# Yixin-F/DR-Using-SCV-OD

Hardware: AMD Instinct MI355X
Metric: scans/sec on SemanticKITTI-seq-05-shaped input (SCV-OD dynamic-removal path, raw scans -> per-point labels + static map) (higher is better)
Workload: dtype f32

## Files before the change

### dr-using-scv-od_amd/csrc/scvod_k_voxels.inc

```
__global__ __launch_bounds__(256) void k_apri_expand(DevParams P, Arena A, int s0) {
    const int s = s0 + blockIdx.y;
    const int base = A.scan_off[s];
    const int n = A.counts[s * 8 + 4];
    for (int i = blockIdx.x * 256 + threadIdx.x; i < n; i += gridDim.x * 256) {
        const float4 q = A.pts[base + A.apri_src[(size_t)base + i]];
        Apri a;
        apri_of_point(P.bin, q.x, q.y, q.z, q.w, a);
        scvod_apri out;
        out.x = a.x;
        out.y = a.y;
        out.z = a.z;
        out.range = a.range;
        out.angle = a.angle;
        out.azimuth = a.azimuth;
        out.intensity = a.intensity;
        out.range_idx = a.range_idx;
        out.sector_idx = a.sector_idx;
        out.azimuth_idx = a.azimuth_idx;
        out.voxel_idx = a.voxel_idx;
        A.apri[(size_t)base + i] = out;
    }
}

__global__ __launch_bounds__(256) void k_cls_from_lists(Arena A, int s) {
    const int base = A.scan_off[s];
    const int n_g = A.counts[s * 8 + 1], n_ng = A.counts[s * 8 + 2];
    for (int i = blockIdx.x * 256 + threadIdx.x; i < n_g + n_ng; i += gridDim.x * 256) {
        if (i < n_g)
            A.cls[base + A.ground_idx[(size_t)base + i]] = SCVOD_CLS_GROUND;
        else
            A.cls[base + A.nonground_idx[(size_t)base + (i - n_g)]] = SCVOD_CLS_NONGROUND;
    }
}

__global__ __launch_bounds__(1024) void k_bin_direct(DevParams P, Arena A, int apply_filter) {
    __shared__ int wsum[17];
    const int s = blockIdx.x;
    const int base = A.scan_off[s];
    const int n = A.scan_off[s + 1] - base;
    int run = 0;
    for (int c0 = 0; c0 < n; c0 += 1024) {
        int i = c0 + threadIdx.x;
        int keep = 0;
        Apri a;
        if (i < n) {
            float4 q = A.pts[base + i];
            keep = apri_of_point(P.bin, q.x, q.y, q.z, q.w, a);
            if (!apply_filter) keep = 1;
        }
        int tk;
        int ek = block_excl_scan<1024>(keep, tk, wsum);
        if (i < n) {
            if (keep) {
                size_t dst = (size_t)base + run + ek;
                scvod_apri out;
                out.x = a.x;
                out.y = a.y;
                out.z = a.z;
                out.range = a.range;
                out.angle = a.angle;
                out.azimuth = a.azimuth;
                out.intensity = a.intensity;
                out.range_idx = a.range_idx;
                out.sector_idx = a.sector_idx;
                out.azimuth_idx = a.azimuth_idx;
                out.voxel_idx = a.voxel_idx;
                A.apri[dst] = out;
                A.apri_src[dst] = i;
                A.apri_key[dst] = a.voxel_idx;
                A.apri_int[dst] = a.intensity;
                A.apri_idx3[dst] = pack_idx3(a.range_idx, a.sector_idx, a.azimuth_idx);
            } else {
                A.rejected_src[(size_t)base + (i - (run + ek))] = i;
            }
        }
        run += tk;
    }
    if (threadIdx.x == 0) {
        A.scan_irr[s] = 0;
        A.irr_list[(size_t)s * (kIrrListCap + 1)] = -1;
        int* c = A.counts + s * 8;
        c[0] = n;
        c[1] = 0;
        c[2] = 0;
        c[3] = 0;
        c[4] = run;
        c[5] = n - run;
        c[6] = 0;
        c[7] = 0;
    }
}

__global__ __launch_bounds__(256) void k_apri_split(Arena A) {
    const int s = blockIdx.y;
    const int base = A.scan_off[s];
    const int n = A.counts[s * 8 + 4];
    for (int i = blockIdx.x * 256 + threadIdx.x; i < n; i += gridDim.x * 256) {
        const scvod_apri& a = A.apri[(size_t)base + i];
        A.apri_key[(size_t)base + i] = a.voxel_idx;
        A.apri_int[(size_t)base + i] = a.intensity;
        A.apri_idx3[(size_t)base + i] = pack_idx3(a.range_idx, a.sector_idx, a.azimuth_idx);
    }
}

__device__ __forceinline__ int vx_bucket_of(const DevParams& P, const Arena& A, int s, int32_t voxel_idx) {
    if (A.vb_lut) {
        if (voxel_idx == 0x7fffffff) return kMaxBuckets - 1;
        return A.vb_lut[(size_t)s * kVgLutBins + (voxel_idx >> *A.vb_lut_shift)];
    }
    int64_t b = ((int64_t)voxel_idx + P.key_off) >> P.vb_shift;
    if (b < 0) b = 0;
    if (b > P.n_buckets - 1) b = P.n_buckets - 1;
    return (int)b;
}
__device__ __forceinline__ uint32_t vx_bias(int32_t k) { return (uint32_t)k ^ 0x80000000u; }
__device__ __forceinline__ int32_t vx_unbias(uint32_t u) { return (int32_t)(u ^ 0x80000000u); }

__global__ __launch_bounds__(1024) void k_vx_partition(DevParams P, Arena A) {
    __shared__ int hist[kMaxBuckets];
    __shared__ int wsum[17];
    const int s = blockIdx.x;
    const int base = A.scan_off[s];
    const int n = A.counts[s * 8 + 4];
    const int tid = threadIdx.x;
    if (tid < kMaxBuckets) hist[tid] = 0;
    __syncthreads();
    constexpr int U = 4;
    for (int i0 = 0; i0 < n; i0 += 1024 * U) {
        int32_t key[U];
#pragma unroll
        for (int u = 0; u < U; ++u) key[u] = A.apri_key[(size_t)base + min(i0 + u * 1024 + tid, n - 1)];
#pragma unroll
        for (int u = 0; u < U; ++u) wave_bin_add(hist, i0 + u * 1024 + tid < n ? vx_bucket_of(P, A, s, key[u]) : -1);
    }
    __syncthreads();
    const int c = (tid < P.n_buckets) ? hist[tid] : 0;
    int total;
    const int ex = block_excl_scan<1024>(c, total, wsum);
    if (tid < kMaxBuckets) {
        A.vb_count[s * kMaxBuckets + tid] = c;
        hist[tid] = ex;
    }
    if (tid <= P.n_buckets) A.vb_off[s * (kMaxBuckets + 1) + tid] = ex;
    __syncthreads();
    for (int i0 = 0; i0 < n; i0 += 1024 * U) {
        int32_t key[U];
#pragma unroll
        for (int u = 0; u < U; ++u) key[u] = A.apri_key[(size_t)base + min(i0 + u * 1024 + tid, n - 1)];
#pragma unroll
        for (int u = 0; u < U; ++u) {
            const int i = i0 + u * 1024 + tid;
            const int bk = i < n ? vx_bucket_of(P, A, s, key[u]) : -1;
            const int at = wave_bin_rank(hist, bk);
            if (bk >= 0) {
                if (A.vx_k32)
                    ((uint32_t*)A.vkeys)[(size_t)base + at] = (uint32_t)((((int64_t)key[u] + P.key_off) & ((1ll << P.vb_shift) - 1)) << A.vx_idx_bits) | (uint32_t)i;
                else
                    A.vkeys[(size_t)base + at] = pack_key(vx_bias(key[u]), (uint32_t)i);
            }
        }
    }
}

#ifndef SCVOD_VOX_K32_LDS
#define SCVOD_VOX_K32_LDS 1
#endif
constexpr size_t vox_key_bytes(int cap, size_t ksize) { return (((size_t)(cap + cap / 8) * (SCVOD_VOX_K32_LDS ? ksize : 8)) + 15) & ~(size_t)15; }
constexpr size_t vox_aux_bytes(int cap, bool desc) { return desc ? (size_t)cap * 4 : ((size_t)(cap / 64) * 4 + 15) & ~(size_t)15; }
constexpr size_t vox_lds_bytes(int cap, size_t ksize = 8, bool desc = true) {
    return vox_key_bytes(cap, ksize) + (size_t)cap * 4 + vox_aux_bytes(cap, desc) + 128;
}
#ifndef SCVOD_VOX_LEAN_MORE
#define SCVOD_VOX_LEAN_MORE 4
#endif
#ifndef SCVOD_VOX_LEAN_S
#define SCVOD_VOX_LEAN_S 12
#endif
template <int U, typename F>
__device__ __forceinline__ void vx_descriptor(int n, F&& at, float& av_out, float& cov_out) {
    float av = 0.f;
    for (int j0 = 0; j0 < n; j0 += U) {
        float x[U];
#pragma unroll
        for (int u = 0; u < U; ++u) x[u] = (j0 + u < n) ? at(j0 + u) : 0.f;
#pragma unroll
        for (int u = 0; u < U; ++u)
            if (j0 + u < n) av += x[u];
    }
    const float fn = (float)n;
    av = av / fn;
    float cov = 0.f;
    for (int j0 = 0; j0 < n; j0 += U) {
        float x[U];
#pragma unroll
        for (int u = 0; u < U; ++u) x[u] = (j0 + u < n) ? at(j0 + u) : 0.f;
#pragma unroll
        for (int u = 0; u < U; ++u)
            if (j0 + u < n) {
                const double d = (double)(x[u] - av);
                cov = (float)((double)cov + d * d);
            }
    }
    av_out = av;
    cov_out = cov / fn;
}
constexpr bool vx_bucket_padfree(int cap) { return SCVOD_VOX_PADFREE == 2 || (SCVOD_VOX_PADFREE == 1 && cap >= 2048); }
template <int CAP, int THREADS, int C_LO, int C_HI, int LGE, int MODE = 0, typename KT = unsigned long long, bool DESC = true>
__global__ __launch_bounds__(THREADS)
#if SCVOD_VOX_K32_LDS
__attribute__((amdgpu_waves_per_eu((sizeof(KT) == 4 && CAP <= 4096 && CAP >= 2048) ? (DESC ? 6 : 2 * SCVOD_VOX_LEAN_MORE) : 1, 8)))
#endif
void k_vx_bucket(DevParams P, Arena A) {
    static_assert(DESC || MODE == 0, "the lean form is makeHashCloud's");
    extern __shared__ __attribute__((aligned(16))) unsigned char smem[];
    constexpr bool K32 = sizeof(KT) == 4;
    constexpr bool PADFREE = vx_bucket_padfree(CAP);
    constexpr bool PADK = true;
    constexpr int SLOTS = CAP + CAP / 8;
    KT* l_keys = (KT*)smem;
    constexpr size_t KB = vox_key_bytes(CAP, sizeof(KT));
    static_assert(KB >= (size_t)SLOTS * sizeof(KT), "key area");
    int* l_vbeg = (int*)(smem + KB);
    float* l_int = (float*)(smem + KB + (size_t)CAP * 4);
    int* wsum = (int*)(smem + KB + (size_t)CAP * 4 + vox_aux_bytes(CAP, DESC));
    int lo, hi;
    order_range(A.vorder_off, C_LO, C_HI, lo, hi);
    constexpr bool PV = (CAP == 4096 && MODE == 0);
    PROF_BEGIN();
    for (int w = lo + blockIdx.x; w < hi; w += gridDim.x) {
    if (PV) PROF_RESET();
    const int4 item = A.vorder[w];
    const int code = item.x;
    const int s = code / kMaxBuckets, b = code - s * kMaxBuckets;
    const int m = item.y;
    const int base = item.z, off = item.w;
    if (MODE == 1 && b == kMaxBuckets - 1) {
        if (threadIdx.x == 0) A.vb_nvox[s * kMaxBuckets + b] = 0;
        continue;
    }
    const bool in_lds = (m <= CAP);
    KT* keys;
    int* vbeg;
    float* ints;
    KT* gkeys = (KT*)A.vkeys + (size_t)base + off;
    const KT kpad = K32 ? (KT)0xffffffffu : (KT)kKeyPad;
    const uint32_t imask = (1u << A.vx_idx_bits) - 1u;
    auto k_major = [&](KT k) -> uint32_t { return K32 ? (uint32_t)k >> A.vx_idx_bits : key_major((unsigned long long)k); };
    auto k_idx = [&](KT k) -> uint32_t { return K32 ? (uint32_t)k & imask : key_idx((unsigned long long)k); };
    if (in_lds) {
        int np2 = 1 << LGE;
        while (np2 < m) np2 <<= 1;
        const int nlive = sortnet::live_end(m, LGE);
        constexpr int IT = CAP / THREADS;
        keys = l_keys;
        vbeg = l_vbeg;
        ints = l_int;
        bool from_regs = false;
        if constexpr (IT == (1 << LGE) && CAP >= 4096) {
            if (np2 == CAP) {
                from_regs = true;
                KT tmp[IT];
                if constexpr (PADFREE) {
                    if ((int)threadIdx.x < (nlive >> LGE)) {
#pragma unroll
                        for (int it = 0; it < IT; ++it) {
                            const int j = sortnet::start_key(it, (int)threadIdx.x, nlive, LGE);
                            tmp[it] = (j < m) ? gkeys[j] : kpad;
                        }
                    }
                    if (PV) PROF_MARK(3, 0);
                    padfree_sort_regs<THREADS, PADK, LGE>(tmp, keys, np2, nlive, kpad);
                } else {
#pragma unroll
                    for (int it = 0; it < IT; ++it) {
                        const int j = it * THREADS + (int)threadIdx.x;
                        tmp[it] = (j < m) ? gkeys[j] : kpad;
                    }
                    if (PV) PROF_MARK(3, 0);
                    block_bitonic_sort_pow2_regs<THREADS, PADK, LGE>(tmp, keys);
                }
            }
        }
        if (!from_regs) {
            const int nfill = PADFREE ? nlive : np2;
            for (int j = threadIdx.x; j < nfill; j += THREADS) l_keys[sort_slot<PADK>(j)] = (j < m) ? gkeys[j] : kpad;
            __syncthreads();
            if (PV) PROF_MARK(3, 0);
            if constexpr (PADFREE)
                padfree_sort<THREADS, PADK, LGE>(keys, np2, nlive, kpad);
            else
                block_bitonic_sort_pow2<THREADS, PADK, LGE>(keys, np2);
        }
        if (PV) PROF_MARK(3, 1);
    } else {
        keys = gkeys;
        vbeg = A.tmp_vox_begin + (size_t)base + off;
        ints = nullptr;
        block_bitonic_sort<THREADS, false>(keys, m);
    }
#define KX(j) (in_lds ? sort_slot<PADK>(j) : (j))
    int run = 0;
    if (in_lds) {
        constexpr int NW = THREADS / 64;
        static_assert(CAP / 64 <= 128, "two (chunk, wave) counts per lane");
        int* wcnt = (int*)l_int;
        const int lane = threadIdx.x & 63, wave = threadIdx.x >> 6;
        const int chunks = (m + THREADS - 1) / THREADS;
        auto head_of = [&](int j, KT& cur) -> bool {
            cur = keys[KX(j)];
            const KT prev = keys[KX(j > 0 ? j - 1 : 0)];
            return (j == 0) || (k_major(cur) != k_major(prev));
        };
        for (int c = 0; c < chunks; ++c) {
            const int j = c * THREADS + threadIdx.x;
            bool head = false;
            if (j < m) {
                KT cur;
                head = head_of(j, cur);
                if (MODE == 0) A.vox_pts[(size_t)base + off + j] = (int32_t)k_idx(cur);
            }
            const unsigned long long hb = __ballot(head);
            if (lane == 0) wcnt[c * NW + wave] = __popcll(hb);
        }
        __syncthreads();
        const int ne = chunks * NW;
        if (wave == 0) {
            const int a0 = (2 * lane < ne) ? wcnt[2 * lane] : 0, a1 = (2 * lane + 1 < ne) ? wcnt[2 * lane + 1] : 0;
            const int inc = wave_incl_scan(a0 + a1);
            if (2 * lane < ne) wcnt[2 * lane] = inc - a0 - a1;
            if (2 * lane + 1 < ne) wcnt[2 * lane + 1] = inc - a1;
            if (lane == 63) wsum[0] = inc;
        }
        __syncthreads();
        run = wsum[0];
        for (int c = 0; c < chunks; ++c) {
            const int j = c * THREADS + threadIdx.x;
            KT cur;
            const bool head = (j < m) && head_of(j, cur);
            const unsigned long long hb = __ballot(head);
            if (head) vbeg[wcnt[c * NW + wave] + __popcll(hb & ((1ull << lane) - 1ull))] = j;
        }
    }
    for (int c0 = 0; c0 < m && !in_lds; c0 += THREADS) {
        int j = c0 + threadIdx.x;
        int head = 0;
        if (j < m) {
            const KT cur = keys[KX(j)];
            const KT prev = keys[KX(j > 0 ? j - 1 : 0)];
            head = (j == 0) || (k_major(cur) != k_major(prev));
            const uint32_t idx = k_idx(cur);
            if (MODE == 0) A.vox_pts[(size_t)base + off + j] = (int32_t)idx;
        }
        int th;
        int eh = block_excl_scan<THREADS>(head, th, wsum);
        if (head) vbeg[run + eh] = j;
        run += th;
    }
    __syncthreads();
    if (PV) PROF_MARK(3, 2);
    const int nv = run;
    if (MODE == 1) {
        float4* tmp = (float4*)A.apri;
        for (int v = threadIdx.x; v < nv; v += THREADS) {
            const int j0 = vbeg[v];
            const int j1 = (v + 1 < nv) ? vbeg[v + 1] : m;
            float sx = 0.f, sy = 0.f, sz = 0.f, si = 0.f;
            for (int j = j0; j < j1; ++j) {
                const float4 p = A.pts[base + k_idx(keys[KX(j)])];
                sx += p.x;
                sy += p.y;
                sz += p.z;
                si += A.vg_labels ? p.w * A.vg_max_intensity : p.w;
            }
            const float fn = (float)(j1 - j0);
            tmp[(size_t)base + off + v] = make_float4(sx / fn, sy / fn, sz / fn, si / fn);
        }
        if (threadIdx.x == 0) A.vb_nvox[s * kMaxBuckets + b] = nv;
        __syncthreads();
        continue;
    }
    auto vox_key_of = [&](int j0) -> int32_t {
        return K32 ? (int32_t)(((int64_t)b << P.vb_shift) + (int64_t)k_major(keys[KX(j0)]) - P.key_off) : vx_unbias(k_major(keys[KX(j0)]));
    };
    if constexpr (DESC) {
        if (in_lds) {
            for (int j = threadIdx.x; j < m; j += THREADS) ints[j] = A.apri_int[(size_t)base + k_idx(keys[KX(j)])];
            __syncthreads();
        }
        if (PV) PROF_MARK(3, 3);
        for (int v = threadIdx.x; v < nv; v += THREADS) {
            const int j0 = vbeg[v];
            const int j1 = (v + 1 < nv) ? vbeg[v + 1] : m;
            float av, cov;
            if (in_lds)
                vx_descriptor<1>(j1 - j0, [&](int j) { return ints[j0 + j]; }, av, cov);
            else
                vx_descriptor<1>(j1 - j0, [&](int j) { return A.apri_int[(size_t)base + k_idx(keys[j0 + j])]; }, av, cov);
            A.tmp_vox_key[(size_t)base + off + v] = vox_key_of(j0);
            A.tmp_vox_cov[(size_t)base + off + v] = cov;
            A.tmp_vox_av[(size_t)base + off + v] = av;
        }
// ... 67 lines not shown
```

### dr-using-scv-od_amd/csrc/scvod_kernels.hip

```cpp
#include <type_traits>

#include "scvod_boxgrid.h"
#include "scvod_grid.h"
#include "scvod_sortnet.h"
#include <rocprim/device/device_radix_sort.hpp>

namespace scvod {

#ifdef SCVOD_PROFILE
__device__ unsigned long long g_prof[8][16];
#define PROF_BEGIN() unsigned long long t_prev = wall_clock64()
#define PROF_RESET()                                   \
    do {                                               \
        __syncthreads();                               \
        if (threadIdx.x == 0) t_prev = wall_clock64(); \
    } while (0)
#define PROF_MARK(k, i)                                      \
    do {                                                     \
        __syncthreads();                                     \
        if (threadIdx.x == 0) {                              \
            const unsigned long long t_now = wall_clock64(); \
            atomicAdd(&g_prof[k][i], t_now - t_prev);        \
            t_prev = t_now;                                  \
        }                                                    \
// ... 196 lines not shown

template <bool PAD, int LGE, typename T>
__device__ __forceinline__ void bitonic_run_to_lds(T (&e)[1 << LGE], T* a, int b) {
    constexpr int E = 1 << LGE;
#pragma unroll
    for (int kk = 2; kk <= E; kk <<= 1) {
#pragma unroll
        for (int d = kk >> 1; d >= 1; d >>= 1) {
#pragma unroll
            for (int m = 0; m < E; ++m)
                if ((m & d) == 0) {
                    if (kk == E || (m & kk) == 0)
                        cswap_asc(e[m], e[m + d]);
                    else
                        cswap_asc(e[m + d], e[m]);
                }
        }
    }
    const int rev = ((b & E) == 0) ? 0 : (E - 1);
#pragma unroll
    for (int m = 0; m < E; ++m) a[sort_slot<PAD>(b + (m ^ rev))] = e[m];
}

template <int THREADS, bool PAD, int LGE, typename T>
__device__ __forceinline__ void block_bitonic_merge_stages(T* a, int np2);

template <int THREADS, bool PAD, int LGE, typename T>
__device__ __forceinline__ void block_bitonic_sort_pow2(T* a, int np2) {
    constexpr int E = 1 << LGE;
    for (int g = threadIdx.x; g < (np2 >> LGE); g += THREADS) {
        const int b = g << LGE;
        T e[E];
#pragma unroll
        for (int m = 0; m < E; ++m) e[m] = a[sort_slot<PAD>(b + m)];
        bitonic_run_to_lds<PAD, LGE>(e, a, b);
    }
    __syncthreads();
    block_bitonic_merge_stages<THREADS, PAD, LGE>(a, np2);
}

template <int THREADS, bool PAD, int LGE, typename T>
__device__ __forceinline__ void block_bitonic_sort_pow2_regs(T (&e)[1 << LGE], T* a) {
    bitonic_run_to_lds<PAD, LGE>(e, a, (int)threadIdx.x << LGE);
    __syncthreads();
    block_bitonic_merge_stages<THREADS, PAD, LGE>(a, THREADS << LGE);
}

template <int THREADS, bool PAD, int LGE, typename T>
__device__ __forceinline__ void block_bitonic_merge_stages(T* a, int np2) {
    constexpr int E = 1 << LGE;
    int lgk = LGE + 1;
    for (int k = 2 * E; k <= np2; k <<= 1, ++lgk) {
        int r = lgk;
        const int first = (r % LGE) ? (r % LGE) : LGE;
        if (first == 1)
            bitonic_pass<THREADS, PAD, 1>(a, np2, k, r);
        else if (first == 2)
            bitonic_pass<THREADS, PAD, 2>(a, np2, k, r);
        else if (first == 3)
            bitonic_pass<THREADS, PAD, 3>(a, np2, k, r);
        else
            bitonic_pass<THREADS, PAD, 4>(a, np2, k, r);
        r -= first;
        while (r > 0) {
            bitonic_pass<THREADS, PAD, LGE>(a, np2, k, r);
            r -= LGE;
        }
    }
}

#ifndef SCVOD_SORT_PADFREE
#define SCVOD_SORT_PADFREE 1
#endif
#ifndef SCVOD_VOX_PADFREE
#define SCVOD_VOX_PADFREE 1
#endif
struct CxAsc {
    template <typename T>
    __device__ __forceinline__ void operator()(T& lo, T& hi) const { cswap_asc(lo, hi); }
};

template <int THREADS, bool PAD, int LT, bool MIRROR, typename T>
__device__ __forceinline__ void padfree_pass(T* a, int np2, int nlive, int r, T padv) {
    const int items = sortnet::pass_items(np2, nlive, r, LT);
    for (int t = threadIdx.x; t < items; t += THREADS) sortnet::pass_item<LT, MIRROR, PAD, T>(a, t, r, nlive, padv, CxAsc{});
    __syncthreads();
}

template <int THREADS, bool PAD, int LGE, typename T>
__device__ __forceinline__ void padfree_merge_stages(T* a, int np2, int nlive, T padv) {
    sortnet::for_each_pass<LGE>(np2, [&](int r, int lt, bool mirror) {
        if (!mirror)
            padfree_pass<THREADS, PAD, LGE, false>(a, np2, nlive, r, padv);
        else if (lt == 1)
            padfree_pass<THREADS, PAD, 1, true>(a, np2, nlive, r, padv);
        else if (lt == 2)
            padfree_pass<THREADS, PAD, 2, true>(a, np2, nlive, r, padv);
        else if (lt == 3 || LGE == 3)
            padfree_pass<THREADS, PAD, 3, true>(a, np2, nlive, r, padv);
        else if constexpr (LGE >= 4)
            padfree_pass<THREADS, PAD, 4, true>(a, np2, nlive, r, padv);
    });
}

template <int THREADS, bool PAD, int LGE, typename T>
__device__ __forceinline__ void padfree_sort(T* a, int np2, int nlive, T padv) {
    constexpr int E = 1 << LGE;
    for (int g = threadIdx.x; g < (nlive >> LGE); g += THREADS) {
        T e[E];
#pragma unroll
        for (int m = 0; m < E; ++m) e[m] = a[sort_slot<PAD>((g << LGE) + m)];
        sortnet::run_store<LGE, PAD>(e, a, g, CxAsc{});
    }
    __syncthreads();
    padfree_merge_stages<THREADS, PAD, LGE>(a, np2, nlive, padv);
}

template <int THREADS, bool PAD, int LGE, typename T>
__device__ __forceinline__ void padfree_sort_regs(T (&e)[1 << LGE], T* a, int np2, int nlive, T padv) {
    if ((int)threadIdx.x < (nlive >> LGE)) sortnet::run_store<LGE, PAD>(e, a, (int)threadIdx.x, CxAsc{});
    __syncthreads();
    padfree_merge_stages<THREADS, PAD, LGE>(a, np2, nlive, padv);
}

#include "scvod_k_patchwork.inc"
#include "scvod_k_voxelgrid.inc"
#include "scvod_k_voxels.inc"
#include "scvod_k_cluster.inc"
#include "scvod_k_merge.inc"
#include "scvod_k_rgrow.inc"
#include "scvod_k_calib.inc"
#include "scvod_k_probe_nn.inc"
#define TH_BEGIN(name) \
    if (th) th(tu, name, 1)
#define TH_END(name) \
    if (th) th(tu, name, 0)

#ifndef SCVOD_SORT_LGE
#define SCVOD_SORT_LGE 4
#endif
constexpr int kLGE = SCVOD_SORT_LGE;
constexpr int kTS = (kLGE == 4) ? 1 : 2;
#ifndef SCVOD_VOX_LGE
#define SCVOD_VOX_LGE 3
#endif
constexpr int kLGEv = SCVOD_VOX_LGE, kTSv = (kLGEv == 4) ? 1 : 2;
constexpr int kPersistCUs = 256;
constexpr int kSortCapS = 1024, kSortThreadsS = 64;
constexpr int kSortCapL = 8192, kSortThreadsL = 512;
constexpr int kSortCapXL = 16384, kClassXL = 52;
constexpr size_t sort_lds_bytes(int cap) { return (size_t)(cap + cap / 8) * 8; }
constexpr int kVoxCapS = 1024, kVoxThreadsS = 64;
constexpr int kVoxCapL = 8192, kVoxThreadsL = 512;

void launch_process(const DevParams& P, const Arena& A, hipStream_t st, int do_patchwork, int apply_filter,
                    int do_voxels, TimerHook th, void* tu, int lean_voxels, int lean_emit) {
    const int B = A.n_scans;
    if (B <= 0) return;
    if (do_patchwork == 1) {
        hipMemsetAsync(A.patch_count, 0, sizeof(int32_t) * (size_t)B * kMaxPatches, st);
        hipMemsetAsync(A.patch_cursor, 0, sizeof(int32_t) * (size_t)B * kMaxPatches, st);
        dim3 gcls((A.max_scan_pts + kClsThreads * kClsItems - 1) / (kClsThreads * kClsItems), B);
        TH_BEGIN("pw_classify");
        hipLaunchKernelGGL(k_pw_classify, gcls, dim3(kClsThreads), 0, st, P, A);
        TH_END("pw_classify");
        TH_BEGIN("pw_offsets");
        hipLaunchKernelGGL(k_pw_offsets, dim3(B), dim3(1024), 0, st, P, A);
        TH_END("pw_offsets");
        TH_BEGIN("pw_scatter");
        hipLaunchKernelGGL(k_pw_scatter, gcls, dim3(kClsThreads), 0, st, P, A);
        TH_END("pw_scatter");
        hipMemsetAsync(A.order_hist, 0, sizeof(int32_t) * 64, st);
        hipMemsetAsync(A.order_cursor, 0, sizeof(int32_t) * 64, st);
        const int n_all = B * P.n_patches;
        TH_BEGIN("pw_order");
        hipLaunchKernelGGL(k_pw_order_count, dim3((n_all + 255) / 256), dim3(256), 0, st, P, A);
        hipLaunchKernelGGL(k_pw_order_offsets, dim3(1), dim3(64), 0, st, A);
        hipLaunchKernelGGL(k_pw_order_scatter, dim3((n_all + 255) / 256), dim3(256), 0, st, P, A);
        TH_END("pw_order");
        hipFuncSetAttribute((const void*)k_pw_sort<kSortCapXL, 1024, kClassXL, 63, 4>, hipFuncAttributeMaxDynamicSharedMemorySize,
                            (int)sort_lds_bytes(kSortCapXL));
        hipFuncSetAttribute((const void*)k_pw_sort<kSortCapL, kSortThreadsL * kTS, kClassL, kClassXL - 1, kLGE>,
                            hipFuncAttributeMaxDynamicSharedMemorySize, (int)sort_lds_bytes(kSortCapL));
        TH_BEGIN("pw_sort_8192");
        hipLaunchKernelGGL((k_pw_sort<kSortCapXL, 1024, kClassXL, 63, 4>), dim3(kPersistCUs), dim3(1024), sort_lds_bytes(kSortCapXL), st, P, A);
        hipLaunchKernelGGL((k_pw_sort<kSortCapL, kSortThreadsL * kTS, kClassL, kClassXL - 1, kLGE>), dim3(kPersistCUs * 2),
                           dim3(kSortThreadsL * kTS), sort_lds_bytes(kSortCapL), st, P, A);
        TH_END("pw_sort_8192");
        TH_BEGIN("pw_sort_4096");
        hipLaunchKernelGGL((k_pw_sort<4096, 256 * kTS, kClassM2, kClassL - 1, kLGE>), dim3(kPersistCUs * 4), dim3(256 * kTS),
                           sort_lds_bytes(4096), st, P, A);
        TH_END("pw_sort_4096");
        TH_BEGIN("pw_sort_2048");
        hipLaunchKernelGGL((k_pw_sort<2048, 128 * kTS, kClassM, kClassM2 - 1, kLGE>), dim3(kPersistCUs * 8), dim3(128 * kTS),
                           sort_lds_bytes(2048), st, P, A);
        TH_END("pw_sort_2048");
        TH_BEGIN("pw_sort_1024");
        hipLaunchKernelGGL((k_pw_sort<kSortCapS, kSortThreadsS * kTS, kClassXS, kClassM - 1, kLGE>), dim3(kPersistCUs * 16),
                           dim3(kSortThreadsS * kTS), sort_lds_bytes(kSortCapS), st, P, A);
        TH_END("pw_sort_1024");
        TH_BEGIN("pw_sort_256");
        hipLaunchKernelGGL((k_pw_sort<256, 64, kClassWave, kClassXS - 1, 3>), dim3(kPersistCUs * 32), dim3(64),
                           sort_lds_bytes(256), st, P, A);
        TH_END("pw_sort_256");
        TH_BEGIN("pw_sort_wave");
        hipLaunchKernelGGL(k_pw_sort_wave, dim3(kPersistCUs * 8), dim3(256), 0, st, P, A);
        TH_END("pw_sort_wave");
        const int coop_class = (B <= 8) ? kClassWave : kClassFitCoop;
        const int coop_min = 1 << (coop_class / 4);
        TH_BEGIN("pw_fit_large");
        const dim3 gfit((int)(A.total_pts / coop_min / (B <= 8 ? 1 : 4)) + 1);
        if (B <= 8) {
            if (lean_emit)
                hipLaunchKernelGGL((k_pw_fit_coop<64, true>), gfit, dim3(64), 0, st, P, A, coop_class);
            else
                hipLaunchKernelGGL((k_pw_fit_coop<64, false>), gfit, dim3(64), 0, st, P, A, coop_class);
        } else {
            if (lean_emit)
                hipLaunchKernelGGL((k_pw_fit_coop<16, true>), gfit, dim3(64), 0, st, P, A, coop_class);
            else
                hipLaunchKernelGGL((k_pw_fit_coop<16, false>), gfit, dim3(64), 0, st, P, A, coop_class);
        }
        TH_END("pw_fit_large");
        TH_BEGIN("pw_fit");
        hipLaunchKernelGGL(k_pw_fit, dim3((n_all + 63) / 64), dim3(64), 0, st, P, A, coop_class);
        TH_END("pw_fit");
        TH_BEGIN("pw_arrange");
        if (lean_emit) {
            if (coop_class > kClassWave) hipLaunchKernelGGL((k_pw_arrange<64, true>), dim3(kPersistCUs * 8), dim3(256), 0, st, P, A, kClassWave, coop_class - 1);
            hipLaunchKernelGGL((k_pw_arrange<16, true>), dim3(kPersistCUs * 4), dim3(256), 0, st, P, A, 0, kClassWave - 1);
        } else {
            if (coop_class > kClassWave) hipLaunchKernelGGL((k_pw_arrange<64, false>), dim3(kPersistCUs * 8), dim3(256), 0, st, P, A, kClassWave, coop_class - 1);
            hipLaunchKernelGGL((k_pw_arrange<16, false>), dim3(kPersistCUs * 4), dim3(256), 0, st, P, A, 0, kClassWave - 1);
        }
        TH_END("pw_arrange");
        TH_BEGIN("emit_offsets");
        hipLaunchKernelGGL(k_emit_offsets, dim3(B), dim3(1024), 0, st, P, A);
        TH_END("emit_offsets");
        TH_BEGIN("emit");
        if (lean_emit)
            hipLaunchKernelGGL(k_emit<true>, dim3(kPersistCUs * 8), dim3(kEmitThreads), 0, st, P, A);
        else
            hipLaunchKernelGGL(k_emit<false>, dim3(kPersistCUs * 8), dim3(kEmitThreads), 0, st, P, A);
        TH_END("emit");
    } else if (do_patchwork == 0) {
        TH_BEGIN("bin_direct");
        hipLaunchKernelGGL(k_bin_direct, dim3(B), dim3(1024), 0, st, P, A, apply_filter);
        TH_END("bin_direct");
    }
    if (do_voxels) {
        if (do_patchwork == 2) {
            hipMemsetAsync(A.scan_irr, 0, sizeof(int32_t) * (size_t)B, st);
            hipMemsetAsync(A.irr_list, 0xff, sizeof(int32_t) * (size_t)B * (kIrrListCap + 1), st);
            hipLaunchKernelGGL(k_apri_split, dim3((A.max_scan_pts + 2047) / 2048, B), dim3(256), 0, st, A);
        }
        TH_BEGIN("vx_partition");
        hipLaunchKernelGGL(k_vx_partition, dim3(B), dim3(1024), 0, st, P, A);
        TH_END("vx_partition");
        dim3 gb(P.n_buckets, B);
        hipMemsetAsync(A.vorder_hist, 0, sizeof(int32_t) * 64, st);
        hipMemsetAsync(A.vorder_cursor, 0, sizeof(int32_t) * 64, st);
        const int nb_all = B * P.n_buckets;
        TH_BEGIN("vx_order");
        hipLaunchKernelGGL(k_vx_order_count, dim3((nb_all + 255) / 256), dim3(256), 0, st, P, A);
        hipLaunchKernelGGL(k_vx_order_offsets, dim3(1), dim3(64), 0, st, A);
        hipLaunchKernelGGL(k_vx_order_scatter, dim3((nb_all + 255) / 256), dim3(256), 0, st, P, A);
        TH_END("vx_order");
        if (do_patchwork == 3) {
            hipFuncSetAttribute((const void*)k_vx_bucket<kVoxCapL, kVoxThreadsL * kTSv, kClassL, 63, kLGEv, 1>,
                                hipFuncAttributeMaxDynamicSharedMemorySize, (int)vox_lds_bytes(kVoxCapL));
            hipFuncSetAttribute((const void*)k_vx_bucket<4096, 256 * kTSv, kClassM2, kClassL - 1, kLGEv, 1>,
                                hipFuncAttributeMaxDynamicSharedMemorySize, (int)vox_lds_bytes(4096));
            hipLaunchKernelGGL((k_vx_bucket<kVoxCapL, kVoxThreadsL * kTSv, kClassL, 63, kLGEv, 1>), dim3(kPersistCUs), dim3(kVoxThreadsL * kTSv),
                               vox_lds_bytes(kVoxCapL), st, P, A);
            hipLaunchKernelGGL((k_vx_bucket<4096, 256 * kTSv, kClassM2, kClassL - 1, kLGEv, 1>), dim3(kPersistCUs * 2), dim3(256 * kTSv),
                               vox_lds_bytes(4096), st, P, A);
            hipLaunchKernelGGL((k_vx_bucket<2048, 128 * kTSv, kClassM, kClassM2 - 1, kLGEv, 1>), dim3(kPersistCUs * 4), dim3(128 * kTSv),
                               vox_lds_bytes(2048), st, P, A);
            hipLaunchKernelGGL((k_vx_bucket<kVoxCapS, kVoxThreadsS * kTSv, kClassXS, kClassM - 1, kLGEv, 1>), dim3(kPersistCUs * 8),
                               dim3(kVoxThreadsS * kTSv), vox_lds_bytes(kVoxCapS), st, P, A);
            hipLaunchKernelGGL((k_vx_bucket<256, 64, 0, kClassXS - 1, 3, 1>), dim3(kPersistCUs * 32), dim3(64), vox_lds_bytes(256), st,
                               P, A);
            hipLaunchKernelGGL(k_vx_final_offsets, dim3(B), dim3(1024), 0, st, P, A);
            return;
        }
        auto bucket_tiers = [&](auto kt, auto desc) {
            using KT = decltype(kt);
            constexpr size_t KS = sizeof(KT);
            constexpr bool DESC = decltype(desc)::value;
            constexpr int kMore = (KS == 4 && SCVOD_VOX_K32_LDS) ? (DESC ? 3 : SCVOD_VOX_LEAN_MORE) : 2;
            hipFuncSetAttribute((const void*)k_vx_bucket<kVoxCapL, kVoxThreadsL * kTSv, kClassL, 63, kLGEv, 0, KT, DESC>,
                                hipFuncAttributeMaxDynamicSharedMemorySize, (int)vox_lds_bytes(kVoxCapL, KS, DESC));
            hipFuncSetAttribute((const void*)k_vx_bucket<4096, 256 * kTSv, kClassM2, kClassL - 1, kLGEv, 0, KT, DESC>,
                                hipFuncAttributeMaxDynamicSharedMemorySize, (int)vox_lds_bytes(4096, KS, DESC));
            TH_BEGIN("vx_bucket_8192");
            hipLaunchKernelGGL((k_vx_bucket<kVoxCapL, kVoxThreadsL * kTSv, kClassL, 63, kLGEv, 0, KT, DESC>), dim3(kPersistCUs), dim3(kVoxThreadsL * kTSv),
                               vox_lds_bytes(kVoxCapL, KS, DESC), st, P, A);
            TH_END("vx_bucket_8192");
            TH_BEGIN("vx_bucket_4096");
            hipLaunchKernelGGL((k_vx_bucket<4096, 256 * kTSv, kClassM2, kClassL - 1, kLGEv, 0, KT, DESC>), dim3(kPersistCUs * kMore), dim3(256 * kTSv),
                               vox_lds_bytes(4096, KS, DESC), st, P, A);
            TH_END("vx_bucket_4096");
            TH_BEGIN("vx_bucket_2048");
            hipLaunchKernelGGL((k_vx_bucket<2048, 128 * kTSv, kClassM, kClassM2 - 1, kLGEv, 0, KT, DESC>), dim3(kPersistCUs * kMore * 2), dim3(128 * kTSv),
                               vox_lds_bytes(2048, KS, DESC), st, P, A);
            TH_END("vx_bucket_2048");
            TH_BEGIN("vx_bucket_1024");
            hipLaunchKernelGGL((k_vx_bucket<kVoxCapS, kVoxThreadsS * kTSv, kClassXS, kClassM - 1, kLGEv, 0, KT, DESC>), dim3(kPersistCUs * (DESC ? 8 : SCVOD_VOX_LEAN_S)),
                               dim3(kVoxThreadsS * kTSv), vox_lds_bytes(kVoxCapS, KS, DESC), st, P, A);
            TH_END("vx_bucket_1024");
            TH_BEGIN("vx_bucket_256");
            hipLaunchKernelGGL((k_vx_bucket<256, 64, 0, kClassXS - 1, 3, 0, KT, DESC>), dim3(kPersistCUs * 32), dim3(64), vox_lds_bytes(256, KS, DESC), st, P, A);
            TH_END("vx_bucket_256");
        };
        if (A.vx_k32) {
            if (lean_voxels)
                bucket_tiers((uint32_t)0, std::false_type{});
            else
                bucket_tiers((uint32_t)0, std::true_type{});
        } else {
            if (lean_voxels)
                bucket_tiers((unsigned long long)0, std::false_type{});
            else
                bucket_tiers((unsigned long long)0, std::true_type{});
        }
        TH_BEGIN("vx_final_offsets");
        hipLaunchKernelGGL(k_vx_final_offsets, dim3(B), dim3(1024), 0, st, P, A);
        TH_END("vx_final_offsets");
        TH_BEGIN("vx_final");
        if (lean_voxels)
            hipLaunchKernelGGL(k_vx_final<false>, dim3((P.n_buckets + 3) / 4, B), dim3(256), 0, st, P, A);
        else
            hipLaunchKernelGGL(k_vx_final<true>, dim3((P.n_buckets + 3) / 4, B), dim3(256), 0, st, P, A);
        TH_END("vx_final");
    }
}

void launch_vox_descriptors(const Arena& A, int s0, int n_scans, hipStream_t st, TimerHook th, void* tu) {
    if (n_scans <= 0 || A.max_scan_pts <= 0) return;
    TH_BEGIN("vx_descriptors");
    hipLaunchKernelGGL(k_vx_descriptors, dim3((A.max_scan_pts + 4095) / 4096, n_scans), dim3(256), 0, st, A, s0);
    TH_END("vx_descriptors");
}

void launch_apri_intensity(const Arena& A, hipStream_t st, TimerHook th, void* tu) {
    if (A.n_scans <= 0 || A.max_scan_pts <= 0) return;
    TH_BEGIN("emit_intensity");
    hipLaunchKernelGGL(k_apri_intensity, dim3((A.max_scan_pts + 2047) / 2048, A.n_scans), dim3(256), 0, st, A);
    TH_END("emit_intensity");
}

void launch_emit_lists(const Arena& A, hipStream_t st, TimerHook th, void* tu) {
    if (A.n_scans <= 0 || A.max_scan_pts <= 0) return;
    TH_BEGIN("emit_lists");
    hipLaunchKernelGGL(k_emit_lists, dim3(kPersistCUs * 8), dim3(kEmitThreads), 0, st, A);
    TH_END("emit_lists");
}

void launch_apri_expand(const DevParams& P, const Arena& A, int s0, int n_scans, int max_pts, hipStream_t st) {
    if (n_scans <= 0 || max_pts <= 0) return;
    hipLaunchKernelGGL(k_apri_expand, dim3((max_pts + 1023) / 1024, n_scans), dim3(256), 0, st, P, A, s0);
}

void launch_voxelgrid_keys(const Arena& A, const VgJob& J, hipStream_t st) {
    const int B = A.n_scans;
    if (B <= 0) return;
    hipMemsetAsync(A.vg_range, 0, sizeof(int32_t), st);
    hipLaunchKernelGGL(k_vg_minmax, dim3(B), dim3(1024), 0, st, A, J);
    if (A.max_scan_pts > 0)
        hipLaunchKernelGGL(k_vg_keys, dim3((A.max_scan_pts + 2047) / 2048, B), dim3(256), 0, st, A, J);
}
void launch_voxelgrid_lut(const Arena& A, hipStream_t st) {
    if (A.n_scans <= 0 || A.max_scan_pts <= 0) return;
    hipFuncSetAttribute((const void*)k_vg_lut, hipFuncAttributeMaxDynamicSharedMemorySize, kVgLutBins * (int)sizeof(int));
    hipLaunchKernelGGL(k_vg_lut, dim3(A.n_scans), dim3(1024), kVgLutBins * sizeof(int), st, A, (int32_t*)A.vb_lut_shift);
}
void launch_voxelgrid_gather(const DevParams& P, const Arena& A, const VgJob& J, long long out_capacity, hipStream_t st) {
    if (A.n_scans <= 0 || A.max_scan_pts <= 0) return;
    hipLaunchKernelGGL(k_vg_outoff, dim3(1), dim3(1024), 0, st, A);
    hipLaunchKernelGGL(k_vg_final, dim3(P.n_buckets, A.n_scans), dim3(256), 0, st, A, J, out_capacity);
}

void launch_cls(const Arena& A, int s, size_t scan_base, int n_points, hipStream_t st) {
    if (n_points <= 0) return;
    hipMemsetAsync(A.cls + scan_base, SCVOD_CLS_DROPPED, (size_t)n_points, st);
    hipLaunchKernelGGL(k_cls_from_lists, dim3((n_points + 2047) / 2048), dim3(256), 0, st, A, s);
}

void launch_cluster(const DevParams& P, const Arena& A0, int from_apri, hipStream_t st, TimerHook th, void* tu) {
    Arena A = A0;
    hipMemsetAsync(A.cc_stats, 0, 8 * sizeof(int32_t), st);
    const int B = A.n_scans;
    if (B <= 0 || A.max_scan_pts <= 0) return;
    A.cc_help_blocks = A.cc_help_blocks_wanted > 0 ? 1 : 0;
    hipMemsetAsync(A.cc_again, 0, sizeof(int32_t), st);
    hipMemsetAsync(A.cc_help, 0, kCcHelpWords * sizeof(int32_t), st);
    hipFuncSetAttribute((const void*)k_cc_scan, hipFuncAttributeMaxDynamicSharedMemorySize, (int)kCcLdsBytes);
    hipFuncSetAttribute((const void*)k_cc_exact, hipFuncAttributeMaxDynamicSharedMemorySize, (int)kCcLdsBytes);
    TH_BEGIN("cc_scan");
    hipLaunchKernelGGL(k_cc_order, dim3(1), dim3(1024), 0, st, A);
    hipLaunchKernelGGL(k_cc_scan, dim3(B), dim3(kCcThreads), kCcLdsBytes, st, P, A, from_apri);
    TH_END("cc_scan");
    TH_BEGIN("cc_exact");
    hipLaunchKernelGGL(k_cc_exact, dim3(kCcExactBlocks), dim3(kCcThreads), kCcLdsBytes, st, P, A, from_apri);
    TH_END("cc_exact");
}

size_t merge_lds_bytes(const DevParams& P, int max_scan_pts) {
    return 4 * ((size_t)P.bin.range_num * P.bin.azimuth_num + 1 + ((size_t)max_scan_pts + 31) / 32);
}

void launch_merge(const DevParams& P, const Arena& A, const MergeJob& M, int from_apri, hipStream_t st, TimerHook th, void* tu) {
    hipMemsetAsync(M.stats, 0, 8 * sizeof(int32_t), st);
    const int B = A.n_scans;
    if (B <= 0 || A.max_scan_pts <= 0) return;
    const size_t lds = merge_lds_bytes(P, A.max_scan_pts);
    hipFuncSetAttribute((const void*)k_im_merge, hipFuncAttributeMaxDynamicSharedMemorySize, (int)lds);
    TH_BEGIN("im_merge");
    hipLaunchKernelGGL(k_im_merge, dim3(B), dim3(kImThreads), lds, st, P, A, M, from_apri);
    TH_END("im_merge");
    TH_BEGIN("im_tables");
    hipLaunchKernelGGL(k_im_tables, dim3(B), dim3(kImThreads), 0, st, P, A, M, from_apri);
    TH_END("im_tables");
}

size_t rg_sort_bytes(int chunk_pts) {
    size_t bytes = 0;
    rocprim::radix_sort_keys(nullptr, bytes, (uint64_t*)nullptr, (uint64_t*)nullptr, (size_t)chunk_pts, 0, 64, (hipStream_t)0);
    return bytes;
}

void launch_rgrow(const DevParams& P, const Arena& A, const RgJob& J, int chunk_pts, void* sort_tmp, size_t sort_bytes, hipStream_t st,
                  TimerHook th, void* tu) {
    if (J.ns <= 0 || chunk_pts <= 0 || A.max_scan_pts <= 0) return;
    int bits = 1;
    while (bits < 31 && (1ll << bits) < chunk_pts) ++bits;
    hipMemsetAsync(J.bmin, 0xff, sizeof(uint32_t) * 3 * (size_t)chunk_pts, st);
    hipMemsetAsync(J.bmax, 0, sizeof(uint32_t) * 3 * (size_t)chunk_pts, st);
    hipMemsetAsync(J.bcnt, 0, sizeof(int32_t) * (size_t)chunk_pts, st);
    hipMemsetAsync(J.key_in, 0xff, sizeof(uint64_t) * (size_t)chunk_pts, st);
    hipMemsetAsync(J.cnt, 0, 2 * sizeof(int32_t), st);
    const dim3 gs((A.max_scan_pts + kRgThreads - 1) / kRgThreads, J.ns);
    const int gp = (chunk_pts + kRgThreads - 1) / kRgThreads;
    TH_BEGIN("rg_select");
    hipLaunchKernelGGL(k_rg_box, gs, dim3(kRgThreads), 0, st, A, J);
    hipLaunchKernelGGL(k_rg_select, gs, dim3(kRgThreads), 0, st, P, A, J);
    TH_END("rg_select");
    TH_BEGIN("rg_sort");
    size_t b = sort_bytes;
    rocprim::radix_sort_keys(sort_tmp, b, J.key_in, J.key_out, (size_t)chunk_pts, 0, 32 + bits + 1, st);
    hipLaunchKernelGGL(k_rg_group, dim3(gp), dim3(kRgThreads), 0, st, A, J);
    TH_END("rg_sort");
    TH_BEGIN("rg_grid");
    hipLaunchKernelGGL(k_rg_grid, dim3(2048), dim3(kRgThreads), 0, st, J);
    TH_END("rg_grid");
    TH_BEGIN("rg_knn");
    hipLaunchKernelGGL(k_rg_knn, dim3(gp), dim3(kRgThreads), 0, st, J);
    TH_END("rg_knn");
    TH_BEGIN("rg_normal");
    hipLaunchKernelGGL(k_rg_normal, dim3(gp), dim3(kRgThreads), 0, st, A, J);
    hipLaunchKernelGGL(k_rg_edges, dim3(gp), dim3(kRgThreads), 0, st, J);
    TH_END("rg_normal");
    TH_BEGIN("rg_grow");
    const size_t lds = sizeof(unsigned long long) * kRgLdsPts;
    hipFuncSetAttribute((const void*)k_rg_grow, hipFuncAttributeMaxDynamicSharedMemorySize, (int)lds);
// ... 146 lines not shown
```

Baseline: 94350.

## Replace sorting network with counting sort for large lean voxel buckets

Adds a counting-sort path to the voxel bucket kernel for 32-bit keys in tiers of 2048 and above, used in lean mode by default. It histograms voxel keys in LDS with atomics, scans the counts to get voxel starts, scatters the keys, and orders points within each voxel by rank counting, instead of running the bitonic sorting network. When a bucket has a voxel denser than a threshold, it falls back to the network sort. The new path needs a larger LDS footprint and a different workgroup count per CU, and it only applies when the bucket shift equals 12.

```diff
diff --git a/dr-using-scv-od_amd/csrc/scvod_k_voxels.inc b/dr-using-scv-od_amd/csrc/scvod_k_voxels.inc
--- a/dr-using-scv-od_amd/csrc/scvod_k_voxels.inc
+++ b/dr-using-scv-od_amd/csrc/scvod_k_voxels.inc
@@ -167,8 +167,29 @@
 #endif
 constexpr size_t vox_key_bytes(int cap, size_t ksize) { return (((size_t)(cap + cap / 8) * (SCVOD_VOX_K32_LDS ? ksize : 8)) + 15) & ~(size_t)15; }
 constexpr size_t vox_aux_bytes(int cap, bool desc) { return desc ? (size_t)cap * 4 : ((size_t)(cap / 64) * 4 + 15) & ~(size_t)15; }
-constexpr size_t vox_lds_bytes(int cap, size_t ksize = 8, bool desc = true) {
-    return vox_key_bytes(cap, ksize) + (size_t)cap * 4 + vox_aux_bytes(cap, desc) + 128;
+#ifndef SCVOD_VOX_COUNT
+#define SCVOD_VOX_COUNT 1
+#endif
+constexpr int kVxCountShift = 12;
+#ifndef SCVOD_VOX_COUNT_DENSE
+#define SCVOD_VOX_COUNT_DENSE 256
+#endif
+constexpr int kVxCountDense = SCVOD_VOX_COUNT_DENSE;
+#ifndef SCVOD_VOX_COUNT_M
+#define SCVOD_VOX_COUNT_M 4
+#endif
+#ifndef SCVOD_VOX_COUNT_L
+#define SCVOD_VOX_COUNT_L 2
+#endif
+constexpr bool vx_bucket_counting(int cap, size_t ksize, int mode, bool desc) {
+    return ksize == 4 && mode == 0 && cap >= 2048 && (SCVOD_VOX_COUNT == 2 || (SCVOD_VOX_COUNT == 1 && !desc));
+}
+constexpr int vx_count_per_cu(int cap, bool desc) { return cap >= 8192 ? 1 : cap >= 4096 ? (desc ? 2 : SCVOD_VOX_COUNT_L) : (desc ? 3 : SCVOD_VOX_COUNT_M); }
+constexpr size_t vox_count_bytes(int cap, bool desc) { return ((size_t)4 << kVxCountShift) + (size_t)(cap + 4) * 4 + (desc ? (size_t)cap * 8 : 0); }
+constexpr size_t vox_lds_bytes(int cap, size_t ksize = 8, bool desc = true, bool count = false) {
+    const size_t net = vox_key_bytes(cap, ksize) + (size_t)cap * 4 + vox_aux_bytes(cap, desc);
+    const size_t cnt = count ? vox_count_bytes(cap, desc) : 0;
+    return (net > cnt ? net : cnt) + 128;
 }
 #ifndef SCVOD_VOX_LEAN_MORE
 #define SCVOD_VOX_LEAN_MORE 4
@@ -204,11 +225,137 @@
     av_out = av;
     cov_out = cov / fn;
 }
+struct VxCountArgs {
+    const uint32_t* gkeys;
+    int32_t* vox_pts;
+    int32_t* out_key;
+    int32_t* out_beg;
+    float* out_av;
+    float* out_cov;
+    const float* apri_int;
+    int32_t* nvox;
+    int32_t key0;
+    int m, off, ib;
+};
+template <int CAP, int THREADS, bool DESC, bool PV>
+__device__ __forceinline__ bool vx_bucket_count(const VxCountArgs& ca
+#ifdef SCVOD_PROFILE
+                                             , unsigned long long& t_prev
+#endif
+) {
+    extern __shared__ __attribute__((aligned(16))) unsigned char smem[];
+    constexpr int SPAN = 1 << kVxCountShift;
+    constexpr int IT = CAP / THREADS;
+    constexpr int CPT = SPAN / THREADS;
+    static_assert(CPT % 4 == 0 && IT % 2 == 0 && CAP <= 8192, "16-byte counter reads; start (13 bits) and count (14) share a word");
+    uint32_t* cnt = (uint32_t*)smem;
+    uint32_t* lst = cnt + SPAN;
+    float* c_int = (float*)(lst + CAP + 4);
+    int* c_vbeg = (int*)(c_int + CAP);
+    int* c_wsum = (int*)(smem + vox_count_bytes(CAP, DESC));
+    const int m = ca.m, ib = ca.ib;
+    const uint32_t imask = (1u << ib) - 1u;
+    for (int i = threadIdx.x; i < SPAN / 4; i += THREADS) ((uint4*)cnt)[i] = make_uint4(0u, 0u, 0u, 0u);
+    uint32_t key[IT];
+#pragma unroll
+    for (int it = 0; it < IT; ++it)
+        key[it] = ca.gkeys[min(it * THREADS + (int)threadIdx.x, m - 1)];
+    __syncthreads();
+    if (PV) PROF_MARK(3, 0);
+    uint32_t arr[IT / 2];
+#pragma unroll
+    for (int it = 0; it < IT; ++it) {
+        uint32_t a = 0u;
+        if (it * THREADS + (int)threadIdx.x < m) a = atomicAdd(&cnt[key[it] >> ib], 1u);
+        if (it & 1)
+            arr[it / 2] |= a << 16;
+        else
+            arr[it / 2] = a;
+    }
+    __syncthreads();
+    if (PV) PROF_MARK(3, 1);
+    const uint4* my_cnt = (const uint4*)cnt + threadIdx.x * (CPT / 4);
+    uint32_t sum = 0, nz = 0, mx = 0;
+#pragma unroll
+    for (int q = 0; q < CPT / 4; ++q) {
+        const uint4 x = my_cnt[q];
+        sum += x.x + x.y + x.z + x.w;
+        nz += (x.x ? 1u : 0u) + (x.y ? 1u : 0u) + (x.z ? 1u : 0u) + (x.w ? 1u : 0u);
+        mx = max(max(mx, max(x.x, x.y)), max(x.z, x.w));
+    }
+    if (__syncthreads_or(mx > (uint32_t)kVxCountDense)) return false;
+    int tot;
+    const int ex = block_excl_scan<THREADS>((int)(sum | (nz << 16)), tot, c_wsum);
+    const int nv = tot >> 16;
+    int start = ex & 0xffff, v = ex >> 16;
+    int32_t vkey = ca.key0 + (int32_t)threadIdx.x * CPT;
+    auto voxel = [&](uint32_t& n) {
+        if (n) {
+            ca.out_key[v] = vkey;
+            ca.out_beg[v] = ca.off + start;
+            if constexpr (DESC) c_vbeg[v] = start;
+            const int first = start;
+            start += (int)n;
+            n = (uint32_t)first | (n << 16);
+            ++v;
+        }
+        ++vkey;
+    };
+#pragma unroll
+    for (int q = 0; q < CPT / 4; ++q) {
+        uint4 x = my_cnt[q];
+        voxel(x.x);
+        voxel(x.y);
+        voxel(x.z);
+        voxel(x.w);
+        ((uint4*)cnt)[threadIdx.x * (CPT / 4) + q] = x;
+    }
+    if (threadIdx.x < 4) lst[m + (int)threadIdx.x] = 0xffffffffu;
+    if (threadIdx.x == 0) *ca.nvox = nv;
+    __syncthreads();
+    if (PV) PROF_MARK(3, 2);
+#pragma unroll
+    for (int it = 0; it < IT; ++it) {
+        if (it * THREADS + (int)threadIdx.x < m)
+            lst[(cnt[key[it] >> ib] & 0xffffu) + ((arr[it / 2] >> ((it & 1) * 16)) & 0xffffu)] = key[it];
+    }
+    __syncthreads();
+    if (PV) PROF_MARK(3, 3);
+    for (int p = threadIdx.x; p < m; p += THREADS) {
+        const uint32_t k = lst[p];
+        const uint32_t sc = cnt[k >> ib];
+        const int end = (int)(sc & 0xffffu) + (int)(sc >> 16);
+        int place = (int)(sc & 0xfffcu);
+        for (int q = place; q < end; q += 4) {
+            const uint4 x = *(const uint4*)(lst + q);
+            place += (int)(x.x < k) + (int)(x.y < k) + (int)(x.z < k) + (int)(x.w < k);
+        }
+        ca.vox_pts[place] = (int32_t)(k & imask);
+        if constexpr (DESC) c_int[place] = ca.apri_int[k & imask];
+    }
+    if constexpr (DESC) {
+        __syncthreads();
+        if (PV) PROF_MARK(3, 4);
+        for (int u = threadIdx.x; u < nv; u += THREADS) {
+            const int j0 = c_vbeg[u];
+            const int j1 = (u + 1 < nv) ? c_vbeg[u + 1] : m;
+            float av, cov;
+            vx_descriptor<1>(j1 - j0, [&](int j) { return c_int[j0 + j]; }, av, cov);
+            ca.out_cov[u] = cov;
+            ca.out_av[u] = av;
+        }
+    } else {
+        if (PV) PROF_MARK(3, 4);
+    }
+    __syncthreads();
+    if (PV) PROF_MARK(3, 5);
+    return true;
+}
 constexpr bool vx_bucket_padfree(int cap) { return SCVOD_VOX_PADFREE == 2 || (SCVOD_VOX_PADFREE == 1 && cap >= 2048); }
-template <int CAP, int THREADS, int C_LO, int C_HI, int LGE, int MODE = 0, typename KT = unsigned long long, bool DESC = true>
+template <int CAP, int THREADS, int C_LO, int C_HI, int LGE, int MODE = 0, typename KT = unsigned long long, bool DESC = true, bool COUNT = false>
 __global__ __launch_bounds__(THREADS)
 #if SCVOD_VOX_K32_LDS
-__attribute__((amdgpu_waves_per_eu((sizeof(KT) == 4 && CAP <= 4096 && CAP >= 2048) ? (DESC ? 6 : 2 * SCVOD_VOX_LEAN_MORE) : 1, 8)))
+__attribute__((amdgpu_waves_per_eu((sizeof(KT) == 4 && CAP <= 4096 && CAP >= 2048) ? (COUNT ? vx_count_per_cu(CAP, DESC) * (THREADS / 64) / 4 : DESC ? 6 : 2 * SCVOD_VOX_LEAN_MORE) : 1, 8)))
 #endif
 void k_vx_bucket(DevParams P, Arena A) {
     static_assert(DESC || MODE == 0, "the lean form is makeHashCloud's");
@@ -247,6 +394,29 @@
     const uint32_t imask = (1u << A.vx_idx_bits) - 1u;
     auto k_major = [&](KT k) -> uint32_t { return K32 ? (uint32_t)k >> A.vx_idx_bits : key_major((unsigned long long)k); };
     auto k_idx = [&](KT k) -> uint32_t { return K32 ? (uint32_t)k & imask : key_idx((unsigned long long)k); };
+    if constexpr (COUNT) {
+        static_assert(vx_bucket_counting(CAP, sizeof(KT), MODE, DESC), "a tier that counts");
+        if (in_lds) {
+            VxCountArgs ca;
+            ca.gkeys = (const uint32_t*)gkeys;
+            ca.vox_pts = A.vox_pts + (size_t)base + off;
+            ca.out_key = A.tmp_vox_key + (size_t)base + off;
+            ca.out_beg = A.tmp_vox_begin + (size_t)base + off;
+            ca.out_av = DESC ? A.tmp_vox_av + (size_t)base + off : nullptr;
+            ca.out_cov = DESC ? A.tmp_vox_cov + (size_t)base + off : nullptr;
+            ca.apri_int = DESC ? A.apri_int + (size_t)base : nullptr;
+            ca.nvox = A.vb_nvox + s * kMaxBuckets + b;
+            ca.key0 = (int32_t)(((int64_t)b << P.vb_shift) - P.key_off);
+            ca.m = m;
+            ca.off = off;
+            ca.ib = A.vx_idx_bits;
+#ifdef SCVOD_PROFILE
+            if (vx_bucket_count<CAP, THREADS, DESC, PV>(ca, t_prev)) continue;
+#else
+            if (vx_bucket_count<CAP, THREADS, DESC, PV>(ca)) continue;
+#endif
+        }
+    }
     if (in_lds) {
         int np2 = 1 << LGE;
         while (np2 < m) np2 <<= 1;
diff --git a/dr-using-scv-od_amd/csrc/scvod_kernels.hip b/dr-using-scv-od_amd/csrc/scvod_kernels.hip
--- a/dr-using-scv-od_amd/csrc/scvod_kernels.hip
+++ b/dr-using-scv-od_amd/csrc/scvod_kernels.hip
@@ -372,6 +372,25 @@
 constexpr size_t sort_lds_bytes(int cap) { return (size_t)(cap + cap / 8) * 8; }
 constexpr int kVoxCapS = 1024, kVoxThreadsS = 64;
 constexpr int kVoxCapL = 8192, kVoxThreadsL = 512;
+
+template <int CAP, int THREADS, int C_LO, int C_HI, int LGE, typename KT, bool DESC>
+static void launch_vx_tier(const DevParams& P, const Arena& A, hipStream_t st, int per_cu_network) {
+    if constexpr (vx_bucket_counting(CAP, sizeof(KT), 0, DESC)) {
+        if (P.vb_shift == kVxCountShift) {
+            constexpr size_t lds = vox_lds_bytes(CAP, sizeof(KT), DESC, true);
+            constexpr int per_cu_counting = vx_count_per_cu(CAP, DESC);
+            static_assert(per_cu_counting > 0 && per_cu_counting * lds <= 160 * 1024, "workgroups per CU of a counting tier");
+            if (CAP >= 4096)
+                hipFuncSetAttribute((const void*)k_vx_bucket<CAP, THREADS, C_LO, C_HI, LGE, 0, KT, DESC, true>, hipFuncAttributeMaxDynamicSharedMemorySize, (int)lds);
+            hipLaunchKernelGGL((k_vx_bucket<CAP, THREADS, C_LO, C_HI, LGE, 0, KT, DESC, true>), dim3(kPersistCUs * per_cu_counting), dim3(THREADS), lds, st, P, A);
+            return;
+        }
+    }
+    constexpr size_t lds = vox_lds_bytes(CAP, sizeof(KT), DESC);
+    if (CAP >= 4096)
+        hipFuncSetAttribute((const void*)k_vx_bucket<CAP, THREADS, C_LO, C_HI, LGE, 0, KT, DESC, false>, hipFuncAttributeMaxDynamicSharedMemorySize, (int)lds);
+    hipLaunchKernelGGL((k_vx_bucket<CAP, THREADS, C_LO, C_HI, LGE, 0, KT, DESC, false>), dim3(kPersistCUs * per_cu_network), dim3(THREADS), lds, st, P, A);
+}
 
 void launch_process(const DevParams& P, const Arena& A, hipStream_t st, int do_patchwork, int apply_filter,
                     int do_voxels, TimerHook th, void* tu, int lean_voxels, int lean_emit) {
@@ -509,28 +528,20 @@
             constexpr size_t KS = sizeof(KT);
             constexpr bool DESC = decltype(desc)::value;
             constexpr int kMore = (KS == 4 && SCVOD_VOX_K32_LDS) ? (DESC ? 3 : SCVOD_VOX_LEAN_MORE) : 2;
-            hipFuncSetAttribute((const void*)k_vx_bucket<kVoxCapL, kVoxThreadsL * kTSv, kClassL, 63, kLGEv, 0, KT, DESC>,
-                                hipFuncAttributeMaxDynamicSharedMemorySize, (int)vox_lds_bytes(kVoxCapL, KS, DESC));
-            hipFuncSetAttribute((const void*)k_vx_bucket<4096, 256 * kTSv, kClassM2, kClassL - 1, kLGEv, 0, KT, DESC>,
-                                hipFuncAttributeMaxDynamicSharedMemorySize, (int)vox_lds_bytes(4096, KS, DESC));
             TH_BEGIN("vx_bucket_8192");
-            hipLaunchKernelGGL((k_vx_bucket<kVoxCapL, kVoxThreadsL * kTSv, kClassL, 63, kLGEv, 0, KT, DESC>), dim3(kPersistCUs), dim3(kVoxThreadsL * kTSv),
-                               vox_lds_bytes(kVoxCapL, KS, DESC), st, P, A);
+            launch_vx_tier<kVoxCapL, kVoxThreadsL * kTSv, kClassL, 63, kLGEv, KT, DESC>(P, A, st, 1);
             TH_END("vx_bucket_8192");
             TH_BEGIN("vx_bucket_4096");
-            hipLaunchKernelGGL((k_vx_bucket<4096, 256 * kTSv, kClassM2, kClassL - 1, kLGEv, 0, KT, DESC>), dim3(kPersistCUs * kMore), dim3(256 * kTSv),
-                               vox_lds_bytes(4096, KS, DESC), st, P, A);
+            launch_vx_tier<4096, 256 * kTSv, kClassM2, kClassL - 1, kLGEv, KT, DESC>(P, A, st, kMore);
             TH_END("vx_bucket_4096");
             TH_BEGIN("vx_bucket_2048");
-            hipLaunchKernelGGL((k_vx_bucket<2048, 128 * kTSv, kClassM, kClassM2 - 1, kLGEv, 0, KT, DESC>), dim3(kPersistCUs * kMore * 2), dim3(128 * kTSv),
-                               vox_lds_bytes(2048, KS, DESC), st, P, A);
+            launch_vx_tier<2048, 128 * kTSv, kClassM, kClassM2 - 1, kLGEv, KT, DESC>(P, A, st, kMore * 2);
             TH_END("vx_bucket_2048");
             TH_BEGIN("vx_bucket_1024");
-            hipLaunchKernelGGL((k_vx_bucket<kVoxCapS, kVoxThreadsS * kTSv, kClassXS, kClassM - 1, kLGEv, 0, KT, DESC>), dim3(kPersistCUs * (DESC ? 8 : SCVOD_VOX_LEAN_S)),
-                               dim3(kVoxThreadsS * kTSv), vox_lds_bytes(kVoxCapS, KS, DESC), st, P, A);
+            launch_vx_tier<kVoxCapS, kVoxThreadsS * kTSv, kClassXS, kClassM - 1, kLGEv, KT, DESC>(P, A, st, DESC ? 8 : SCVOD_VOX_LEAN_S);
             TH_END("vx_bucket_1024");
             TH_BEGIN("vx_bucket_256");
-            hipLaunchKernelGGL((k_vx_bucket<256, 64, 0, kClassXS - 1, 3, 0, KT, DESC>), dim3(kPersistCUs * 32), dim3(64), vox_lds_bytes(256, KS, DESC), st, P, A);
+            launch_vx_tier<256, 64, 0, kClassXS - 1, 3, KT, DESC>(P, A, st, 32);
             TH_END("vx_bucket_256");
         };
         if (A.vx_k32) {
```

Result: faster. 97150, median of 6 (+3.0%).
